# EvolvingLMMs-Lab/multimodal-sae

Measured on AMD Instinct MI355X. Metric: tokens/sec through SAE encode+TopK+decode, d=4096 width=131072, higher is better.
Workload: dtype int8 MFMA candidate select + f32 exact re-score/decode (outputs f32-exact); 1 GPU; BASELINE configs[1]: d_model=4096 width=131072 k=32, T=8192 bf16 activations/step resident in HBM, random-init unit-norm f32 weights; k=32, parallelism=single GPU, distinct_batches=4

## Files before the change

### multimodal-sae_amd/csrc/encode_fused.hip

```cpp
#include <new>
#include <cstddef>
#include <cstdlib>
#include <type_traits>

#include "common.h"
#include "gemm_mfma.h"
#include "gemm_skinny.h"
#include "encode_defs.h"
#include "encode_prep.h"
#include "encode_rescore.h"
#include "encode_small.h"
#include "encode_cert.h"

int msae_pre_acts_launch(const void *x, int x_dtype, const float *W_enc, const float *b_enc,
                         const float *b_dec, const int *rows, const int *n_rows, int T, int d, int N,
                         int relu, float *out, int ld_out, hipStream_t s);
int msae_topk_launch(const float *latents, int T, int N, int k, int ld, const int *n_rows,
                     float *vals, int32_t *idx, hipStream_t s, const TopkExtra &ex = TopkExtra());
bool msae_kth_value_launch(const float *rows, int T, int S, int ld, int r, float *out, int out_ld,
                           int out_col, hipStream_t s, const KthPush &push = KthPush());

namespace {

using GemmBf16 = GemmCfg<256, 256, 2, 2, 4, false>;
constexpr int kGemmI8Shape = MSAE_GEMM_MF == 16 ? 128 : 0;
using GemmI8 = GemmCfg<256, 256, 2, 2, 4, true, kGemmI8Shape>;
using GemmI8Cert = GemmCfg<256, 256, 2, 2, 4, true, 32 | kGemmI8Shape>;
using GemmF8 = GemmCfg<256, 256, 2, 2, 4, false, 64>;
constexpr int G_BM = GemmBf16::BM;

__global__ void zero3_i32_kernel(int *p0, size_t n0, int *p1, size_t n1, int *p2, size_t n2) {
  for (size_t i = (size_t)blockIdx.x * 256 + threadIdx.x; i < n0; i += (size_t)gridDim.x * 256) p0[i] = 0;
  for (size_t i = (size_t)blockIdx.x * 256 + threadIdx.x; i < n1; i += (size_t)gridDim.x * 256) p1[i] = 0;
  for (size_t i = (size_t)blockIdx.x * 256 + threadIdx.x; i < n2; i += (size_t)gridDim.x * 256) p2[i] = 0;
}

__global__ void zero_i32_kernel(int *p, size_t n) {
  for (size_t i = (size_t)blockIdx.x * 256 + threadIdx.x; i < n; i += (size_t)gridDim.x * 256) p[i] = 0;
}

__global__ void edit_dense_kernel(float *dense, int ld, int rows, const int *n_rows, int set_feature,
                                  float set_value, int zero_feature) {
  const int r = blockIdx.x * 256 + threadIdx.x;
  const int R = n_rows ? min(rows, *n_rows) : rows;
  if (r >= R) return;
  if (set_feature >= 0) dense[(size_t)r * ld + set_feature] = set_value;
  if (zero_feature >= 0) dense[(size_t)r * ld + zero_feature] = 0.f;
}

__global__ void iota_list_kernel(int *list, int T, int n_total) {
  const int i = blockIdx.x * 256 + threadIdx.x;
  if (i < n_total) list[i] = i < T ? i : (i == T ? T : 0);
}

__global__ void fallback_counts_kernel(const int *n_flagged, int fb_cap, int chunks, int *counts) {
  const int nf = *n_flagged;
  for (int c = threadIdx.x; c < chunks; c += blockDim.x) {
    const int left = nf - c * fb_cap;
    counts[c] = left < 0 ? 0 : (left > fb_cap ? fb_cap : left);
  }
}

struct ShardOut { unsigned char *recs; int C; int row_offset; };

constexpr int PROF_MARKS = 7;
struct ProfState {
  unsigned magic = 0x50524F46u;
  int max_steps = 0, step = 0;
  hipEvent_t *ev = nullptr;
};

inline void prof_mark(ProfState *pf, int i, hipStream_t s) {
  if (pf && pf->step < pf->max_steps) (void)hipEventRecord(pf->ev[pf->step * PROF_MARKS + i], s);
}
inline void prof_step(ProfState *pf) {
  if (pf && pf->step < pf->max_steps) ++pf->step;
}

struct FusedPlan {
  bool fast, i8, small, fm, f8;
  size_t off_fmcount, off_fmtarget, off_fmkeys, off_fmpairs, off_fmpre, off_fmdefer;
  size_t off_xhi, off_xlo, off_skeys, off_sviol, off_surv, off_sbound, off_scand, off_stau;
  int Tp, S, r, cap, r_max, fb_cap, fb_chunks;
  size_t off_rowe, off_cds, off_cds_s, off_cds_p;
  size_t off_xq, off_xqo, off_rowc, off_refs, off_colc, off_colc_s, off_colc_p, off_colmax, off_odims, off_isout, off_wqo, off_wqos;
  size_t off_xb, off_a32, off_sample, off_tauv, off_taui, off_cnt, off_cand, off_segcnt, off_segcand, off_flag, off_fbdense, off_dense, bytes;
  int segs;
};

inline FusedPlan make_plan(int T, int d, int N, int k, int mode, int shard_C = 0, bool cert = false) {
  FusedPlan p{};
  p.fast = fast_shape_ok(N, d) && T > EXACT_T_MAX && k <= 256 && k >= 1;
  if (cert && !cert_shape_ok(N, d)) p.fast = false;
  if (cert) mode = 1;
  size_t o = 0;
  auto take = [&](size_t b) { size_t at = o; o += msae_align_up(b, 256); return at; };
  if (p.fast) {
    p.Tp = (T + G_BM - 1) / G_BM * G_BM;
    p.S = N / SAMPLE_STRIDE;
    p.r = k / 8 > 16 ? k / 8 : 16;
    if (k < 32) p.r = k / 2 > 8 ? k / 2 : 8;
    if (shard_C > 0) { const int rs = shard_C / 8 > 8 ? shard_C / 8 : 8; if (rs < p.r) p.r = rs; }
    p.cap = next_pow2(128 * p.r);
    p.i8 = mode == 1 && i8_shape_ok(N, d);
    p.f8 = mode == 2 && i8_shape_ok(N, d);
    p.small = !cert && p.i8 && small_shape_ok(T, d, N, k) && getenv("MSAE_NO_SMALL_PATH") == nullptr;
    p.r_max = k <= 64 ? 8 * k : 3 * k;
    if (p.r_max < k + 4) p.r_max = k + 4;
    if (p.r_max > p.cap) p.r_max = p.cap;
    if (p.i8 || p.f8) {
      p.off_colc = take((size_t)N * 16);
      p.off_colc_s = take((size_t)p.S * 16);
      p.off_colc_p = take(p.i8 ? (size_t)N * 16 : 0);
      p.off_colmax = take((size_t)d * 4 * COLMAX_PARTS);
      p.off_odims = take((size_t)(MAX_OUT + 1) * 4);
      p.off_isout = take((size_t)d);
    }
    if (p.i8) {
      p.off_xq = take((size_t)p.Tp * d * (cert ? 2 : 1));
      p.off_xqo = take((size_t)p.Tp * MAX_OUT);
      p.off_wqo = take((size_t)N * MAX_OUT);
      p.off_wqos = take((size_t)p.S * MAX_OUT);
    }
    p.off_rowc = take((size_t)p.Tp * 16);
    p.off_rowe = take(p.i8 ? (size_t)p.Tp * 8 : 0);
    p.off_cds = take(p.i8 ? (size_t)N * 4 : 0);
    p.off_cds_s = take(p.i8 ? (size_t)p.S * 4 : 0);
    p.off_cds_p = take(p.i8 ? (size_t)N * 4 : 0);
    p.off_refs = take(256);
    if (p.small) {
      p.off_xhi = take((size_t)T * d);
      p.off_xlo = take((size_t)T * d);
      p.off_skeys = take((size_t)T * 128 * 8);
      p.off_surv = take((size_t)T * SMALL_SURV * 8);
      p.off_sbound = take((size_t)T * SMALL_GRID * 4);
      p.off_scand = take((size_t)T * 128 * 8);
      p.off_stau = take((size_t)T * 4);
      p.off_sviol = take((size_t)T * 2 * 4);
    }
    p.off_xb = take(p.i8 ? 256 : (size_t)p.Tp * d * (p.f8 ? 1 : 2));
    p.off_a32 = take((size_t)T * d * 4);
    p.off_sample = take((size_t)T * p.S * 4);
    const size_t tau_n = (size_t)T * p.r;
    p.off_tauv = take(tau_n * 4);
    p.off_taui = take(tau_n * 4);
    p.off_cnt = take((size_t)T * 4);
    p.segs = (T <= 256 && p.cap >= 1024) ? 8 : 1;
    p.off_segcnt = take(p.segs > 1 ? (size_t)T * p.segs * 4 : 0);
    p.off_cand = take((size_t)T * p.cap * 8);
    p.off_segcand = take(p.segs > 1 ? (size_t)T * p.cap * 8 : 0);
    p.fb_cap = fallback_capacity(T, N);
    p.fb_chunks = (T + p.fb_cap - 1) / p.fb_cap;
    p.off_flag = take(((size_t)T + 64 + p.fb_chunks) * 4);
    p.off_fbdense = take((size_t)p.fb_cap * N * 4);
    p.fm = shard_C == 0 && fm_shape_ok(T, k, N, d, p.r_max);
    if (p.fm) {
      p.off_fmcount = take(((size_t)N + 64 + (N + FM_SCAN_BLOCK - 1) / FM_SCAN_BLOCK) * 4);
      p.off_fmtarget = take((size_t)T * 4);
      p.off_fmkeys = take((size_t)T * p.r_max * 8);
      p.off_fmpairs = take(((size_t)T * p.r_max + (size_t)N * 16) * 8);
      p.off_fmpre = take((size_t)T * p.r_max * 4);
      p.off_fmdefer = take((size_t)T * 2 * 4);
    }
  } else {
    p.off_dense = take((size_t)T * N * 4);
  }
  p.bytes = o;
  return p;
}


template <int DT>
int run_exact_rows(const void *x, const float *W_enc, const float *b_enc, const float *b_dec, const int *list,
                   const int *n_list, int *pass_counts, float *dense, int fb_cap, int fb_chunks, int d, int N, int k,
                   int set_feature, float set_value, int zero_feature, float *vals, IdxOut idx, int32_t *status,
                   int detail, hipStream_t s) {
  if (fb_chunks > 1)
    hipLaunchKernelGGL(fallback_counts_kernel, dim3(1), dim3(64), 0, s, n_list, fb_cap, fb_chunks, pass_counts);
  for (int c = 0; c < fb_chunks; ++c) {
    const int *rows = list + (size_t)c * fb_cap, *n_rows = fb_chunks > 1 ? pass_counts + c : n_list;
    int rc = msae_pre_acts_launch(x, DT, W_enc, b_enc, b_dec, rows, n_rows, fb_cap, d, N, 1, dense, N, s);
    if (rc) return rc;
    if (set_feature >= 0 || zero_feature >= 0)
      hipLaunchKernelGGL(edit_dense_kernel, dim3((fb_cap + 255) / 256), dim3(256), 0, s, dense, N, fb_cap, n_rows,
                         set_feature, set_value, zero_feature);
    TopkExtra ex;
    ex.idx64 = idx.i64; ex.row_map = rows; ex.status = status; ex.detail = detail;
    rc = msae_topk_launch(dense, fb_cap, N, k, N, n_rows, vals, idx.i32, s, ex);
    if (rc) return rc;
  }
  return 0;
}

template <int DT>
int run_exact_fallback(const void *x, const float *W_enc, const float *b_enc, const float *b_dec, int T, int d, int N,
// ... 215 lines not shown
    hipLaunchKernelGGL(gather_wo_kernel, dim3(N / 32), dim3(256), 0, s, wq, N, d, odims,
                       reinterpret_cast<const f32x4 *>(prepared + pp.off_wstat), wqo, wqos, cc_main, cc_samp, cc_perm,
                       skip_sample ? 1 : 0, sd ? reinterpret_cast<const float *>(prepared + pp.off_ds) : (const float *)nullptr,
                       reinterpret_cast<float *>(ws + pl.off_cds), reinterpret_cast<float *>(ws + pl.off_cds_s),
                       reinterpret_cast<float *>(ws + pl.off_cds_p));
    colc = cc_main; colc_s = cc_samp;
    op_main.A = reinterpret_cast<const unsigned char *>(xq); op_main.ldA = d;
    op_main.B = skinny ? prepared + pp.off_wqf : tile_major ? prepared + pp.off_wqp : reinterpret_cast<const unsigned char *>(wq);
    op_main.ldB = d;
    op_main.nk = tile_major == 2 ? d / 64 : d / 128;
    op_main.packed = skinny ? 3 : tile_major;
    op_main.Ao = reinterpret_cast<const unsigned char *>(xqo);
    op_main.Bo = reinterpret_cast<const unsigned char *>(wqo);
    op_main.n_out = odims + MAX_OUT;
    op_samp = op_main;
    op_samp.B = skinny ? prepared + pp.off_wqsf : tile_major ? prepared + pp.off_wqsp : reinterpret_cast<const unsigned char *>(wqs);
    op_samp.Bo = reinterpret_cast<const unsigned char *>(wqos);
    if constexpr (msae_tuning::ABL_NOLEAD) { op_main.Ao = nullptr; op_main.Bo = nullptr; }
  } else if (pl.f8) {
    signed char *x8 = reinterpret_cast<signed char *>(xb);
    unsigned *colmax = reinterpret_cast<unsigned *>(ws + pl.off_colmax);
    int *odims = reinterpret_cast<int *>(ws + pl.off_odims);
    unsigned char *is_out = ws + pl.off_isout;
    f32x4 *cc_main = reinterpret_cast<f32x4 *>(ws + pl.off_colc), *cc_samp = reinterpret_cast<f32x4 *>(ws + pl.off_colc_s);
    const int ychunks = T >= 32 ? (T / 16 < 512 ? T / 16 : 512) : 1;
    hipLaunchKernelGGL((prep_colmax_kernel<DT, true>), dim3((d / 4 + 255) / 256, ychunks), dim3(256), 0, s, x, b_dec, T, d, a32,
                       colmax);
    hipLaunchKernelGGL(pick_outliers_kernel, dim3(1), dim3(1024), 0, s, colmax, d, odims, is_out);
    hipLaunchKernelGGL(quant_x_fp8_kernel, dim3(pl.Tp), dim3(256), 0, s, (const float *)a32, T, d, (const unsigned char *)is_out, x8,
                       rowc, z * z, valid);
    hipLaunchKernelGGL(gather_wo_fp8_kernel, dim3(N / 32), dim3(256), 0, s, W_enc, N, d, (const int *)odims,
                       reinterpret_cast<const f32x4 *>(prepared + pp.off_colbf), cc_main, cc_samp);
    colc = cc_main; colc_s = cc_samp;
    op_main.A = reinterpret_cast<const unsigned char *>(x8); op_main.ldA = d;
    op_main.B = prepared + pp.off_wq; op_main.ldB = d;
    op_main.nk = d / 128;
    op_main.packed = 1;
    op_samp = op_main;
    op_samp.B = prepared + pp.off_wqsp;
  } else {
    hipLaunchKernelGGL(row_p4_kernel, dim3(T), dim3(256), 0, s, a32, T, d, rowc, z * z, valid);
    colc = reinterpret_cast<const f32x4 *>(prepared + pp.off_colbf);
    colc_s = reinterpret_cast<const f32x4 *>(prepared + pp.off_colbf_s);
    op_main.A = reinterpret_cast<const unsigned char *>(xb); op_main.ldA = (size_t)d * 2;
    op_main.B = reinterpret_cast<const unsigned char *>(wb); op_main.ldB = (size_t)d * 2;
    op_main.nk = d / 64;
    op_samp = op_main;
    op_samp.B = reinterpret_cast<const unsigned char *>(wsamp);
  }

  float *refs = reinterpret_cast<float *>(ws + pl.off_refs);
  hipLaunchKernelGGL(band_refs_kernel, dim3(1), dim3(1024), 0, s, colc_s, pl.S, refs);
  prof_mark(co.prof, 1, s);
  {
    GemmEpilogue ep{};
    ep.bias = b_enc; ep.bias_stride = SAMPLE_STRIDE; ep.bias_off = SAMPLE_OFF;
    ep.dense = sample; ep.ld_dense = pl.S;
    ep.rowc = rowc; ep.colc = colc_s; ep.refs = refs; ep.zz12 = zzx;
    if (sd) { ep.row_e = reinterpret_cast<const int2 *>(ws + pl.off_rowe); ep.col_ds = reinterpret_cast<const float *>(ws + pl.off_cds_s); }
    const int grc = skinny == 64    ? gemm_skinny_launch<64, true>(op_samp, T, d, pl.S, ep, s)
                    : skinny == 128 ? gemm_skinny_launch<128, true>(op_samp, T, d, pl.S, ep, s)
                    : skinny == 256 ? gemm_skinny_launch<256, true>(op_samp, T, d, pl.S, ep, s)
                    : pl.i8         ? gemm_launch<GemmI8, true>(op_samp, T, pl.Tp, pl.S, ep, s)
                    : pl.f8         ? gemm_launch<GemmF8, true>(op_samp, T, pl.Tp, pl.S, ep, s)
                                    : gemm_launch<GemmBf16, true>(op_samp, T, pl.Tp, pl.S, ep, s);
    if (grc) return grc;
  }
  prof_mark(co.prof, 2, s);
  int rc = 0;
  const int skip_a = set_feature >= 0 ? set_feature : -1, skip_b = zero_feature >= 0 ? zero_feature : -1;
  KthPush push{};
  bool pushed = false;
  if (skip_sample && skip_a < 0 && skip_b < 0) {
    push.cnt = pcnt; push.cand = pcand; push.cap = seg_cap; push.stride = SAMPLE_STRIDE; push.off = SAMPLE_OFF;
    push.cnt_stride = pl.segs; push.row_stride = pl.cap;
    pushed = true;
  }
  if (!msae_kth_value_launch(sample, T, pl.S, pl.S, pl.r, tauv, pl.r, pl.r - 1, s, push)) {
    rc = msae_topk_launch(sample, T, pl.S, pl.r, pl.S, nullptr, tauv, taui, s);
    if (rc) return rc;
    pushed = false;
  }
  if (skip_sample && !pushed)
    hipLaunchKernelGGL(sample_push_kernel, dim3(T), dim3(256), 0, s, sample, pl.S, tauv, pl.r, pl.r - 1, skip_a, skip_b, pcnt,
                       pcand, seg_cap, pl.segs, pl.cap);
  prof_mark(co.prof, 3, s);
  const int N_main = skip_sample ? N - pl.S : N;
  {
    GemmEpilogue ep{};
    ep.bias = b_enc; ep.bias_stride = 1; ep.bias_off = 0;
    if (skip_sample) { ep.skip_stride = SAMPLE_STRIDE; ep.skip_off = SAMPLE_OFF; }
    ep.tau_vals = tauv; ep.tau_ld = pl.r; ep.tau_col = pl.r - 1;
    ep.cnt = pcnt; ep.cand = pcand; ep.cap = pl.cap; ep.segs = pl.segs;
    ep.skip_a = set_feature >= 0 ? set_feature : -1;
    ep.skip_b = zero_feature >= 0 ? zero_feature : -1;
    ep.rowc = rowc; ep.colc = skip_sample ? cc_perm : colc; ep.refs = refs; ep.zz12 = zzx;
    if (sd) {
      ep.row_e = reinterpret_cast<const int2 *>(ws + pl.off_rowe);
      ep.col_ds = reinterpret_cast<const float *>(ws + (skip_sample ? pl.off_cds_p : pl.off_cds));
    }
    if constexpr (msae_tuning::GEMM_TIMELINE != 0) {
      if (!g_timeline) (void)hipMalloc(&g_timeline, 64 * 8 * 8);
      (void)hipMemsetAsync(g_timeline, 0, 64 * 8 * 8, s);
      ep.timeline = g_timeline;
    }
    const int grc = skinny == 64    ? gemm_skinny_launch<64, false>(op_main, T, d, N_main, ep, s)
                    : skinny == 128 ? gemm_skinny_launch<128, false>(op_main, T, d, N_main, ep, s)
                    : skinny == 256 ? gemm_skinny_launch<256, false>(op_main, T, d, N_main, ep, s)
                    : pl.i8         ? gemm_launch<GemmI8, false>(op_main, T, pl.Tp, N_main, ep, s)
                    : pl.f8         ? gemm_launch<GemmF8, false>(op_main, T, pl.Tp, N, ep, s)
                                    : gemm_launch<GemmBf16, false>(op_main, T, pl.Tp, N, ep, s);
    if (grc) return grc;
  }
  if (pl.segs > 1)
    hipLaunchKernelGGL(compact_candidates_kernel, dim3(T), dim3(64), 0, s, pcnt, pcand, pl.segs, pl.cap, cnt, cand);
  prof_mark(co.prof, 4, s);
  if (shard) {
    PackArgs pa{};
    pa.cnt = cnt; pa.cand = cand; pa.cap = pl.cap;
    pa.tau_vals = tauv; pa.tau_ld = pl.r; pa.tau_col = pl.r - 1;
    pa.rowc = rowc; pa.colc = colc; pa.zz12 = zzx; pa.i8 = (pl.i8 || pl.f8) ? 1 : 0;
    pa.C = shard->C; pa.row_offset = shard->row_offset; pa.stride = shard_record_bytes(shard->C);
    pa.recs = shard->recs;
    if (pl.cap <= 64 * 32) hipLaunchKernelGGL(pack_candidates_kernel<32>, dim3(T), dim3(64), 0, s, pa);
    else if (pl.cap <= 64 * 64) hipLaunchKernelGGL(pack_candidates_kernel<64>, dim3(T), dim3(64), 0, s, pa);
    else return MSAE_ENOTIMPL;
    prof_mark(co.prof, 5, s);
    prof_mark(co.prof, 6, s);
    prof_step(co.prof);
    return msae_launch_status();
  }
// ... 561 lines not shown
```

### multimodal-sae_amd/csrc/gemm_mfma.h

```cpp
#pragma once
#include <cstdlib>

#include "common.h"
#include "tuning.h"


struct GemmEpilogue {
  const float *bias;
  int bias_stride, bias_off;
  int skip_stride, skip_off;
  float *dense; int ld_dense;
  const float *tau_vals; int tau_ld, tau_col;
  int *cnt; unsigned long long *cand; int cap;
  int segs;
  int skip_a, skip_b;
  const f32x4 *rowc, *colc;
  const float *refs;
  float zz12;
  const int2 *row_e;
  const float *col_ds;
  unsigned long long *timeline;
};

struct GemmOperands {
  const unsigned char *A, *B;
  size_t ldA, ldB;
  int nk;
  const unsigned char *Ao, *Bo;
  const int *n_out;
  int packed;
  int cert;
};

constexpr int gemm_side_bytes(int nt) { return 7 * nt * 4; }

template <bool I8_, bool F8_, bool CERT_, bool MF16_>
struct GemmEpiCfg {
  static constexpr bool I8 = I8_, F8 = F8_, CERT = CERT_, MF16 = MF16_;
  static_assert(!(I8 && F8), "fp8 accumulates in f32");
  static_assert(!MF16 || I8, "16x16x64 is an int8 shape");
  static constexpr bool SCALED = I8 || F8;
  static constexpr int BR = MF16 ? 64 : 32, BC = MF16 ? 16 : 32;
  static __device__ __forceinline__ int acc_row(int i, int e, int lane) {
    return i * BR + (MF16 ? 16 * (e >> 2) + 4 * (lane >> 4) + (e & 3) : (e & 3) + 8 * (e >> 2) + 4 * (lane >> 5));
  }
  static __device__ __forceinline__ int acc_col(int j, int lane) { return j * BC + (lane & (BC - 1)); }
};

template <int BM_, int BN_, int STAGES_, int WM_, int WN_, bool I8_ = false, int FLAGS_ = 0>
struct GemmCfg : GemmEpiCfg<I8_, (FLAGS_ & 64) != 0, (FLAGS_ & 32) != 0, (FLAGS_ & 128) != 0> {
  using GemmCfg::GemmEpiCfg::MF16;
  using GemmCfg::GemmEpiCfg::BR;
  using GemmCfg::GemmEpiCfg::BC;
  static constexpr int BM = BM_, BN = BN_, STAGES = STAGES_, WM = WM_, WN = WN_;
  static constexpr bool ABL_NOSTAGE = FLAGS_ & 4, ABL_NOREAD = FLAGS_ & 8, ABL_NOMFMA = FLAGS_ & 16;
  static constexpr int NWAVES = WM * WN, NT = NWAVES * 64;
  static constexpr int TM = BM / WM, TN = BN / WN, MI = TM / BR, NI = TN / BC;
  static constexpr int FA = MF16 ? TM / 16 : MI, FB = MF16 ? TN / 16 : NI;
  static constexpr int ROWB = 128;
  static constexpr int KS = MF16 ? 2 : 4;
  static constexpr int A_BYTES = BM * ROWB, B_BYTES = BN * ROWB, STAGE_BYTES = A_BYTES + B_BYTES;
  static constexpr int LDS_RING_BYTES = STAGES * STAGE_BYTES;
  static constexpr int SIDE_BYTES = gemm_side_bytes(NT);
  static constexpr int QCAP = 2296;
  static constexpr int LDS_BYTES = LDS_RING_BYTES + SIDE_BYTES + 16 + QCAP * 8;
  static_assert(STAGES == 2, "the flat cross-tile k-sequence below is written for a 2-slot ring");
  static_assert(BM + BN <= NT, "one thread per tile row and column fetches the epilogue constants");
  static constexpr int PIECES = STAGE_BYTES / 1024, PPW = PIECES / NWAVES;
  static constexpr int A_PIECES = A_BYTES / 1024;
  static_assert(PIECES % NWAVES == 0, "stage must split evenly over the waves");
  static_assert(TM % BR == 0 && TN % BC == 0 && TM % 32 == 0 && TN % 16 == 0, "tile shape");
  static_assert(LDS_BYTES <= 160 * 1024, "LDS budget");
};

// ... 449 lines not shown
    if constexpr (!DENSE) {
      float c5 = 0.f;
      if (tid < C::BM) {
        float b2 = r.c3 * r.ref0;
        if constexpr (C::SCALED) {
          const float rz = r.c1 * r.c1 * zz12;
          b2 = __builtin_fmaf(rz * r.c4 * r.c4, r.ref2, __builtin_fmaf(rz, r.ref1, b2));
        }
        c5 = __builtin_sqrtf(b2) * 1.00001f;
      } else if (tid < C::BM + C::BN) {
        const float q = __int_as_float(r.c2);
        float h2 = q / r.ref0;
        if constexpr (C::SCALED) {
          h2 = fmaxf(h2, r.c3 / r.ref1);
          if (r.c4 > 0.f) h2 = fmaxf(h2, r.c4 / r.ref2);
        }
        c5 = (q > 0.f || r.c3 > 0.f || r.c4 > 0.f) ? __builtin_sqrtf(h2) * 1.00001f : 0.f;
      }
      s[5 * C::NT + tid] = c5;
    }
  }
};

template <class C>
__device__ __forceinline__ float gemm_band_sq(const GemmSideView<C> &side, int row, int col, float zz12) {
  const float pz = side.P(row);
  if constexpr (!C::SCALED) return pz * side.Q(col);
  const float rs = side.sx(row), mf = side.m(row);
  const float rz = rs * rs * zz12;
  return __builtin_fmaf(pz, side.Q(col), __builtin_fmaf(rz * mf * mf, side.So(col), rz * side.Si(col)));
}

typedef float f32x2 __attribute__((ext_vector_type(2)));
template <class V>
__device__ __forceinline__ V gemm_splat(float x) {
  if constexpr (sizeof(V) == sizeof(float)) return x;
  else return V{x, x};
}
template <class C, class V>
__device__ __forceinline__ V gemm_value(const f32x16 &blk, int e, V sx, float sw, float nds, float bias) {
  V a;
  if constexpr (sizeof(V) == sizeof(float)) {
    if constexpr (C::I8) a = (float)__builtin_bit_cast(i32x16, blk)[e]; else a = blk[e];
  } else {
    if constexpr (C::I8) a = V{(float)__builtin_bit_cast(i32x16, blk)[e], (float)__builtin_bit_cast(i32x16, blk)[e + 1]};
    else a = V{blk[e], blk[e + 1]};
  }
  if constexpr (C::I8 && !C::CERT)
    return __builtin_elementwise_fma(__builtin_elementwise_fma(a, gemm_splat<V>(sw), gemm_splat<V>(nds)), sx, gemm_splat<V>(bias));
  else if constexpr (C::SCALED) return a * (sx * sw) + bias;
  else return a + bias;
}

template <class C, bool DENSE>
__device__ __forceinline__ void gemm_epilogue(f32x16 (&acc)[C::MI][C::NI], const GemmEpilogue &ep, int T,
                                              int m0, int n0, int wr, int wc, int lane,
                                              unsigned char *smem, const GemmSideView<C> side, int tl_tile = 0) {
  constexpr int QCAP = C::QCAP;
  unsigned *q_count = reinterpret_cast<unsigned *>(smem + C::LDS_RING_BYTES + C::SIDE_BYTES);
  unsigned long long *queue = reinterpret_cast<unsigned long long *>(smem + C::LDS_RING_BYTES + C::SIDE_BYTES + 16);
  asm volatile("s_waitcnt lgkmcnt(0)" ::: "memory");
  __builtin_amdgcn_s_barrier();
  if constexpr (!DENSE) {
    if (threadIdx.x == 0) *q_count = 0u;
    __syncthreads();
  }
  MSAE_TL(7);
  float c_bias[C::NI], c_sw[C::NI], c_h[C::NI];
  float c_ds[C::NI];
  bool c_live[C::NI];
#pragma unroll
  for (int j = 0; j < C::NI; ++j) {
    const int col = wc * C::TN + C::acc_col(j, lane);
    c_bias[j] = side.bias(col);
    c_sw[j] = side.sw(col);
    c_ds[j] = (C::I8 && !C::CERT) ? -side.Ds(col) : 0.f;
    c_h[j] = side.h(col);
    const int feat = gemm_feature(ep, n0 + col);
    c_live[j] = (feat != ep.skip_a) && (feat != ep.skip_b);
  }
  if (msae_tuning::ABL_NOEPI && !DENSE && ep.cap != -12345) { asm volatile("" ::"v"(acc[0][0][0])); } else
  if constexpr (!DENSE) {
    unsigned hits[C::MI][C::NI];
    constexpr int RG = C::MF16 ? 4 : 16;
#pragma unroll
    for (int i = 0; i < C::MI; ++i) {
      unsigned mj[C::NI];
#pragma unroll
      for (int j = 0; j < C::NI; ++j) mj[j] = 0u;
#pragma unroll
      for (int g = 0; g < 16 / RG; ++g) {
        if constexpr (RG < 16) __builtin_amdgcn_sched_barrier(0);
        float tau[RG], rs[RG], bt[RG];
#pragma unroll
        for (int r = 0; r < RG; ++r) {
          const int row = wr * C::TM + C::acc_row(i, RG * g + r, lane);
          tau[r] = side.tau(row);
          rs[r] = C::SCALED ? side.sx(row) : 0.f;
          bt[r] = side.B(row);
        }
#pragma unroll
        for (int j = 0; j < C::NI; ++j) {
          unsigned m = mj[j];
#pragma unroll
          for (int r = 0; r < RG; r += 2) {
            const int e = RG * g + r;
// ... 9 lines not shown
          mj[j] = m;
          if (g == 16 / RG - 1) hits[i][j] = c_live[j] ? (~m & 0xFFFFu) : 0u;
        }
      }
      if constexpr (RG < 16) __builtin_amdgcn_sched_barrier(0);
    }
    unsigned total = 0;
#pragma unroll
    for (int i = 0; i < C::MI; ++i)
#pragma unroll
      for (int j = 0; j < C::NI; ++j) total += (unsigned)__builtin_popcount(hits[i][j]);
    if (total) {
      unsigned slot;
      {
        const unsigned qa = (unsigned)(size_t)(__attribute__((address_space(3))) unsigned *)q_count;
        asm volatile("ds_add_rtn_u32 %0, %1, %2\n\ts_waitcnt lgkmcnt(0)" : "=v"(slot) : "v"(qa), "v"(total) : "memory");
      }
#pragma unroll
      for (int i = 0; i < C::MI; ++i) {
#pragma unroll
        for (int j = 0; j < C::NI; ++j) {
          unsigned h = hits[i][j];
          const int col = wc * C::TN + C::acc_col(j, lane);
          while (h) {
            const int p = 31 - __builtin_clz(h);
            h &= ~(1u << p);
            const int e = 15 - p;
            const unsigned b0 = 0u - (e & 1), b1 = 0u - ((e >> 1) & 1), b2 = 0u - ((e >> 2) & 1), b3 = 0u - ((e >> 3) & 1);
            auto sel = [](unsigned mk, unsigned hi, unsigned lo) { return (hi & mk) | (lo & ~mk); };
            unsigned s8[8], s4[4], s2[2];
#pragma unroll
            for (int q = 0; q < 8; ++q) s8[q] = sel(b0, __float_as_uint(acc[i][j][2 * q + 1]), __float_as_uint(acc[i][j][2 * q]));
#pragma unroll
            for (int q = 0; q < 4; ++q) s4[q] = sel(b1, s8[2 * q + 1], s8[2 * q]);
#pragma unroll
            for (int q = 0; q < 2; ++q) s2[q] = sel(b2, s4[2 * q + 1], s4[2 * q]);
            const float v = __uint_as_float(sel(b3, s2[1], s2[0]));
            const int row = wr * C::TM + C::acc_row(i, e, lane);
            if (slot < QCAP) {
              queue[slot] = ((unsigned long long)__float_as_uint(v) << 32) | (unsigned)(row << 16 | col);
            } else {
              const float u = v + __builtin_sqrtf(gemm_band_sq<C>(side, row, col, ep.zz12));
              if (u > side.tau(row)) {
                const int t = m0 + row;
                const int feat = gemm_feature(ep, n0 + col);
                gemm_push_candidate(ep, t, ((unsigned long long)f32_order_key(u) << 32) | (unsigned)(0x7FFFFFFF - feat));
              }
            }
            ++slot;
          }
        }
      }
    }
  } else {
#pragma unroll
    for (int i = 0; i < C::MI; ++i) {
#pragma unroll
      for (int j = 0; j < C::NI; ++j) {
        const int col = wc * C::TN + C::acc_col(j, lane);
#pragma unroll
        for (int e = 0; e < 16; ++e) {
          const int row = wr * C::TM + C::acc_row(i, e, lane), t = m0 + row;
          const float v = gemm_value<C, float>(acc[i][j], e, C::SCALED ? side.sx(row) : 0.f, c_sw[j], c_ds[j], c_bias[j]);
          if (t < T) ep.dense[(size_t)t * ep.ld_dense + n0 + col] = v + __builtin_sqrtf(gemm_band_sq<C>(side, row, col, ep.zz12));
        }
      }
    }
  }
  MSAE_TL(4);
  if constexpr (!DENSE) {
    __syncthreads();
    const unsigned nq = msae_tuning::ABL_NOFLUSH ? 0u : (*q_count < QCAP ? *q_count : QCAP);
    for (unsigned q = threadIdx.x; q < nq; q += C::NT) {
      const unsigned long long e = queue[q];
      const int row = (int)((e >> 16) & 0xFFFFu), col = (int)(e & 0xFFFFu);
      const float v = __uint_as_float((unsigned)(e >> 32));
      const float u = v + __builtin_sqrtf(gemm_band_sq<C>(side, row, col, ep.zz12));
      if (!(u > side.tau(row))) continue;
      const int t = m0 + row;
      const int feat = gemm_feature(ep, n0 + col);
      gemm_push_candidate(ep, t, ((unsigned long long)f32_order_key(u) << 32) | (unsigned)(0x7FFFFFFF - feat));
    }
  }
  MSAE_TL(5);
}

template <class C, bool DENSE>
__global__ __launch_bounds__(C::NT) void gemm_kernel(GemmOperands op, int T, int Tp, int N, int nM, int nN,
                                                     GemmEpilogue ep) {
  extern __shared__ __attribute__((aligned(1024))) unsigned char smem[];
  int seq = 0;
  [[maybe_unused]] int tl_tile = -1;
  for (int tile_id = blockIdx.x; tile_id < nM * nN; tile_id += gridDim.x) {
  ++tl_tile;
  MSAE_TL(0);
  int tid_ = threadIdx.x;
  asm volatile("" : "+v"(tid_));
  const int lane = tid_ & 63;
  const int wave = __builtin_amdgcn_readfirstlane(tid_ >> 6);
  const int wr = wave / C::WN, wc = wave % C::WN;
  int tm, tn;
  gemm_map_tile(tile_id, nM, nN, tm, tn);
  const int m0 = tm * C::BM, n0 = tn * C::BN;
  const bool has_next = tile_id + (int)gridDim.x < nM * nN;
  int m0n = 0, n0n = 0;
  if (has_next) {
// ... 171 lines not shown
```

### multimodal-sae_amd/csrc/topk.hip

```cpp
#include "common.h"

namespace {

constexpr int TK_THREADS = 1024;
constexpr int TK_WAVES = TK_THREADS / 64;
constexpr int TK_BINS = 4096;

struct TkShared {
  unsigned hist[TK_BINS];
  unsigned wave_tot[TK_WAVES];
  unsigned bin;
  unsigned remaining;
  unsigned base_gt;
  unsigned base_eq;
};

__device__ __forceinline__ unsigned wave_incl_scan(unsigned v, int lane) {
#pragma unroll
  for (int off = 1; off < 64; off <<= 1) {
    unsigned n = __shfl_up(v, off, 64);
    if (lane >= off) v += n;
  }
  return v;
}
// ... 192 lines not shown
  {
    unsigned mx = 0u;
#pragma unroll
    for (int i = 0; i < VPL; ++i) mx = key[i] > mx ? key[i] : mx;
#pragma unroll
    for (int off = 32; off > 0; off >>= 1) { const unsigned o = __shfl_xor(mx, off, 64); mx = o > mx ? o : mx; }
    const unsigned pre = mx & 0xFF000000u;
    int c = 0;
#pragma unroll
    for (int i = 0; i < VPL; ++i) c += (key[i] >= pre) ? 1 : 0;
#pragma unroll
    for (int off = 32; off > 0; off >>= 1) c += __shfl_xor(c, off, 64);
    if (c >= r) { lo = pre; first_bit = 23; }
  }
#pragma unroll 1
  for (int bit = first_bit; bit >= KTH_LOW_BIT; --bit) {
    const unsigned mid = lo | (1u << bit);
    int c = 0;
#pragma unroll
    for (int i = 0; i < VPL; ++i) c += (key[i] >= mid) ? 1 : 0;
#pragma unroll
    for (int off = 32; off > 0; off >>= 1) c += __shfl_xor(c, off, 64);
    if (c >= r) lo = mid;
  }
  if (lane == 0) out[(size_t)t * out_ld + out_col] = f32_from_order_key(lo);
  if (push.cnt && f32_from_order_key(lo) > 0.f) {
    int total = 0;
#pragma unroll
    for (int i = 0; i < VPL; ++i) {
      total += __builtin_popcountll(__builtin_amdgcn_ballot_w64(key[i] > lo));
      if ((i & 7) == 7) asm volatile("" : "+s"(total));
    }
    if (total == 0) return;
    int base = 0;
    if (lane == 0) base = atomicAdd(push.cnt + (size_t)t * push.cnt_stride, total);
    base = __builtin_amdgcn_readfirstlane(base);
    unsigned long long *list = push.cand + (size_t)t * (push.row_stride ? push.row_stride : push.cap);
    unsigned lo2 = lo;
    asm volatile("" : "+v"(lo2));
#pragma unroll
    for (int i = 0; i < VPL; ++i) {
      const bool hit = key[i] > lo2;
      const unsigned long long m = __builtin_amdgcn_ballot_w64(hit);
      if (m == 0ull) continue;
      if (hit) {
        const int slot = base + (int)__builtin_amdgcn_mbcnt_hi((unsigned)(m >> 32), __builtin_amdgcn_mbcnt_lo((unsigned)m, 0u));
        const int j = ((i >> 2) * 64 + lane) * 4 + (i & 3);
        unsigned kk;
        asm volatile("v_mov_b32 %0, %1" : "=v"(kk) : "v"(key[i]));
        if (slot < push.cap) list[slot] = ((unsigned long long)kk << 32) | (unsigned)(0x7FFFFFFF - (j * push.stride + push.off));
      }
      base += __builtin_popcountll(m);
      if ((i & 7) == 7) asm volatile("" : "+s"(base));
    }
  }
}

__global__ __launch_bounds__(64) void merge_topk_kernel(const int32_t *__restrict__ gathered, int T,
                                                        int G, int kl, int k,
                                                        float *__restrict__ vals,
                                                        int32_t *__restrict__ idx,
                                                        int32_t *__restrict__ flagged) {
  extern __shared__ __attribute__((aligned(16))) unsigned long long mkeys[];
  const int lane = threadIdx.x, t = blockIdx.x;
  const int M = G * kl, np = next_pow2(M);
  unsigned long long worst_last = 0ull;
  for (int i = lane; i < np; i += 64) {
    unsigned long long key = 0ull;
    if (i < M) {
      const int g = i / kl, j = i % kl;
      const float v = __int_as_float(gathered[(((size_t)g * 2 + 0) * T + t) * kl + j]);
      const int f = gathered[(((size_t)g * 2 + 1) * T + t) * kl + j];
      key = rank_key(v, f);
      if (j == kl - 1) worst_last = key > worst_last ? key : worst_last;
    }
    mkeys[i] = key;
  }
#pragma unroll
  for (int off = 32; off > 0; off >>= 1) {
    const unsigned long long o = __shfl_xor(worst_last, off, 64);
    worst_last = o > worst_last ? o : worst_last;
  }
  for (int size = 2; size <= np; size <<= 1)
    for (int stride = size >> 1; stride > 0; stride >>= 1) {
      __syncthreads();
      for (int i = lane; i < (np >> 1); i += 64) {
        const int lo = (i / stride) * (stride << 1) + (i % stride), hi = lo + stride;
        const bool desc = ((lo & size) == 0);
        const unsigned long long x = mkeys[lo], y = mkeys[hi];
        if ((x < y) == desc) { mkeys[lo] = y; mkeys[hi] = x; }
      }
    }
  __syncthreads();
  for (int j = lane; j < k; j += 64) {
    const unsigned long long key = mkeys[j];
    idx[(size_t)t * k + j] = rank_key_index(key);
    vals[(size_t)t * k + j] = f32_from_order_key((unsigned)(key >> 32));
  }
  if (lane == 0 && flagged) flagged[t] = (kl < k && worst_last >= mkeys[k - 1]) ? 1 : 0;
}

__global__ __launch_bounds__(1024) void compact_flags_kernel(const int32_t *__restrict__ flags, int T,
                                                             int32_t *__restrict__ rows, int32_t *__restrict__ n_rows) {
  __shared__ int wsum[16];
  __shared__ int s_base;
  const int tid = threadIdx.x, lane = tid & 63, wv = tid >> 6;
// ... 44 lines not shown
        const bool desc = ((lo & size) == 0);
        const unsigned long long x = mkeys[lo], y = mkeys[hi];
        if ((x < y) == desc) { mkeys[lo] = y; mkeys[hi] = x; }
      }
    }
  __syncthreads();
  for (int j = lane; j < k; j += 64) {
    const unsigned long long key = mkeys[j];
    if (idx) idx[(size_t)t * k + j] = rank_key_index(key);
    if (idx64) idx64[(size_t)t * k + j] = rank_key_index(key);
    vals[(size_t)t * k + j] = f32_from_order_key((unsigned)(key >> 32));
  }
}

}

extern "C" size_t msae_topk_ws_bytes(int T, int N, int k) {
  (void)T; (void)N; (void)k;
  return 0;
}

int msae_topk_launch(const float *latents, int T, int N, int k, int ld, const int *n_rows,
                     float *vals, int32_t *idx, hipStream_t s, const TopkExtra &ex) {
  if (T < 0 || N <= 0 || k <= 0 || k > N || k > 16384 || ld < N) return MSAE_EINVAL;
  if (T == 0) return 0;
  const size_t smem = sizeof(TkShared) + (size_t)next_pow2(k) * sizeof(unsigned long long);
  const bool vec = (N % 4 == 0) && (ld % 4 == 0) && msae_aligned(latents, 16);
  if (smem > 48 * 1024) {
    if (vec) MSAE_HIP_TRY(hipFuncSetAttribute((const void *)topk_rows_kernel<true>, hipFuncAttributeMaxDynamicSharedMemorySize, (int)smem));
    else MSAE_HIP_TRY(hipFuncSetAttribute((const void *)topk_rows_kernel<false>, hipFuncAttributeMaxDynamicSharedMemorySize, (int)smem));
  }
  const int grid = (n_rows && T > 128) ? 128 : T;
  if (vec)
    hipLaunchKernelGGL(topk_rows_kernel<true>, dim3(grid), dim3(TK_THREADS), smem, s, latents, T, N, k, ld,
                       n_rows, vals, idx, ex);
  else
    hipLaunchKernelGGL(topk_rows_kernel<false>, dim3(grid), dim3(TK_THREADS), smem, s, latents, T, N, k,
                       ld, n_rows, vals, idx, ex);
  return msae_launch_status();
}

bool msae_kth_value_launch(const float *rows, int T, int S, int ld, int r, float *out, int out_ld,
                           int out_col, hipStream_t s, const KthPush &push) {
  if (S % 256 || ld % 4 || !msae_aligned(rows, 16) || r < 1 || r > S) return false;
  const dim3 grid((T + 3) / 4), block(256);
  switch (S / 64) {
#define KTH_CASE(V) case V: hipLaunchKernelGGL(kth_value_kernel<V>, grid, block, 0, s, rows, T, S, ld, r, out, out_ld, out_col, push); return true;
    KTH_CASE(4) KTH_CASE(8) KTH_CASE(16) KTH_CASE(32) KTH_CASE(64) KTH_CASE(128)
#undef KTH_CASE
    default: return false;
  }
}

extern "C" int msae_topk_f32(const float *latents, int T, int N, int k, float *vals, int32_t *idx,
                             void *ws, size_t ws_bytes, void *stream) {
  (void)ws; (void)ws_bytes;
  return msae_topk_launch(latents, T, N, k, N, nullptr, vals, idx, (hipStream_t)stream, TopkExtra());
}

extern "C" int msae_merge_topk(const int32_t *gathered, int T, int G, int kl, int k, float *vals,
                               int32_t *idx, int32_t *flagged, void *stream) {
  if (T < 0 || G <= 0 || kl <= 0 || k <= 0 || (long)G * kl < k || (long)G * kl > 8192) return MSAE_EINVAL;
  if (T == 0) return 0;
  const size_t smem = (size_t)next_pow2(G * kl) * sizeof(unsigned long long);
  MSAE_HIP_TRY(hipFuncSetAttribute((const void *)merge_topk_kernel,
                                   hipFuncAttributeMaxDynamicSharedMemorySize, (int)smem));
  hipLaunchKernelGGL(merge_topk_kernel, dim3(T), dim3(64), smem, (hipStream_t)stream, gathered, T, G,
                     kl, k, vals, idx, flagged);
  return msae_launch_status();
}

extern "C" int msae_compact_flags(const int32_t *flags, int T, int32_t *rows, int32_t *n_rows, void *stream) {
  if (T < 0 || !rows || !n_rows || (T > 0 && !flags)) return MSAE_EINVAL;
  hipLaunchKernelGGL(compact_flags_kernel, dim3(1), dim3(1024), 0, (hipStream_t)stream, flags, T, rows, n_rows);
  return msae_launch_status();
}

extern "C" int msae_merge_topk_masked(const int32_t *gathered, int T, int G, int kl, int k, const int32_t *mask,
                                      float *vals, int32_t *idx, int64_t *idx64, void *stream) {
  if (T < 0 || G <= 0 || kl <= 0 || k <= 0 || (long)G * kl < k || (long)G * kl > 8192 || !mask || !vals || (!idx && !idx64))
    return MSAE_EINVAL;
  if (T == 0) return 0;
  const size_t smem = (size_t)next_pow2(G * kl) * sizeof(unsigned long long);
  MSAE_HIP_TRY(hipFuncSetAttribute((const void *)merge_topk_masked_kernel,
                                   hipFuncAttributeMaxDynamicSharedMemorySize, (int)smem));
  hipLaunchKernelGGL(merge_topk_masked_kernel, dim3(T), dim3(64), smem, (hipStream_t)stream, gathered, T, G, kl, k, mask,
                     vals, idx, idx64);
  return msae_launch_status();
}
```

Before: 1.578 million tokens/s.

## Compact per-tile top-R keys in sample GEMM epilogue instead of dense sample matrix

In the int8 sample GEMM epilogue, each 256-column tile now does a radix select per row. It writes only the top-R keys plus a bound on the discarded keys, instead of storing the full dense sample row. A new kth_compact kernel then selects the r-th threshold from the compacted keys, clamps it by the max discarded bound, and pushes candidates. This cuts the dense sample write and the later full read and select. The cost is extra LDS staging and syncthreads inside the GEMM epilogue, and a threshold that may be looser than before.

```diff
diff --git a/multimodal-sae_amd/csrc/encode_fused.hip b/multimodal-sae_amd/csrc/encode_fused.hip
--- a/multimodal-sae_amd/csrc/encode_fused.hip
+++ b/multimodal-sae_amd/csrc/encode_fused.hip
@@ -19,6 +19,8 @@
                      float *vals, int32_t *idx, hipStream_t s, const TopkExtra &ex = TopkExtra());
 bool msae_kth_value_launch(const float *rows, int T, int S, int ld, int r, float *out, int out_ld,
                            int out_col, hipStream_t s, const KthPush &push = KthPush());
+bool msae_kth_compact_launch(const unsigned long long *ktop, const unsigned *kbound, int T, int n_tiles, int R, int r, float *out,
+                             int out_ld, int out_col, hipStream_t s, const KthPush &push);
 
 namespace {
 
@@ -86,6 +88,8 @@
   size_t off_xq, off_xqo, off_rowc, off_refs, off_colc, off_colc_s, off_colc_p, off_colmax, off_odims, off_isout, off_wqo, off_wqos;
   size_t off_xb, off_a32, off_sample, off_tauv, off_taui, off_cnt, off_cand, off_segcnt, off_segcand, off_flag, off_fbdense, off_dense, bytes;
   int segs;
+  size_t off_ktop, off_kbound;
+  int kR;
 };
 
 inline FusedPlan make_plan(int T, int d, int N, int k, int mode, int shard_C = 0, bool cert = false) {
@@ -141,6 +145,10 @@
     p.off_xb = take(p.i8 ? 256 : (size_t)p.Tp * d * (p.f8 ? 1 : 2));
     p.off_a32 = take((size_t)T * d * 4);
     p.off_sample = take((size_t)T * p.S * 4);
+    p.kR = p.r <= 16 ? 16 : (p.r <= 32 ? 32 : 0);
+    if (!p.i8 || cert || p.S % 256 || p.S / 256 * p.kR > 1024) p.kR = 0;
+    p.off_ktop = take(p.kR ? (size_t)T * (p.S / 256) * p.kR * 8 : 0);
+    p.off_kbound = take(p.kR ? (size_t)T * (p.S / 256) * 4 : 0);
     const size_t tau_n = (size_t)T * p.r;
     p.off_tauv = take(tau_n * 4);
     p.off_taui = take(tau_n * 4);
@@ -462,10 +470,16 @@
   float *refs = reinterpret_cast<float *>(ws + pl.off_refs);
   hipLaunchKernelGGL(band_refs_kernel, dim3(1), dim3(1024), 0, s, colc_s, pl.S, refs);
   prof_mark(co.prof, 1, s);
+  const int skip_a = set_feature >= 0 ? set_feature : -1, skip_b = zero_feature >= 0 ? zero_feature : -1;
+  const bool compact = GemmI8::MF16 && pl.i8 && pl.kR > 0 && skinny == 0 && skip_sample && skip_a < 0 && skip_b < 0 &&
+                       getenv("MSAE_DENSE_SAMPLE") == nullptr;
+  unsigned long long *ktop = reinterpret_cast<unsigned long long *>(ws + pl.off_ktop);
+  unsigned *kbound = reinterpret_cast<unsigned *>(ws + pl.off_kbound);
   {
     GemmEpilogue ep{};
     ep.bias = b_enc; ep.bias_stride = SAMPLE_STRIDE; ep.bias_off = SAMPLE_OFF;
     ep.dense = sample; ep.ld_dense = pl.S;
+    if (compact) { ep.ktop = ktop; ep.kbound = kbound; ep.ktop_r = pl.kR; }
     ep.rowc = rowc; ep.colc = colc_s; ep.refs = refs; ep.zz12 = zzx;
     if (sd) { ep.row_e = reinterpret_cast<const int2 *>(ws + pl.off_rowe); ep.col_ds = reinterpret_cast<const float *>(ws + pl.off_cds_s); }
     const int grc = skinny == 64    ? gemm_skinny_launch<64, true>(op_samp, T, d, pl.S, ep, s)
@@ -478,7 +492,6 @@
   }
   prof_mark(co.prof, 2, s);
   int rc = 0;
-  const int skip_a = set_feature >= 0 ? set_feature : -1, skip_b = zero_feature >= 0 ? zero_feature : -1;
   KthPush push{};
   bool pushed = false;
   if (skip_sample && skip_a < 0 && skip_b < 0) {
@@ -486,7 +499,9 @@
     push.cnt_stride = pl.segs; push.row_stride = pl.cap;
     pushed = true;
   }
-  if (!msae_kth_value_launch(sample, T, pl.S, pl.S, pl.r, tauv, pl.r, pl.r - 1, s, push)) {
+  if (compact) {
+    if (!msae_kth_compact_launch(ktop, kbound, T, pl.S / 256, pl.kR, pl.r, tauv, pl.r, pl.r - 1, s, push)) return MSAE_EINVAL;
+  } else if (!msae_kth_value_launch(sample, T, pl.S, pl.S, pl.r, tauv, pl.r, pl.r - 1, s, push)) {
     rc = msae_topk_launch(sample, T, pl.S, pl.r, pl.S, nullptr, tauv, taui, s);
     if (rc) return rc;
     pushed = false;
diff --git a/multimodal-sae_amd/csrc/gemm_mfma.h b/multimodal-sae_amd/csrc/gemm_mfma.h
--- a/multimodal-sae_amd/csrc/gemm_mfma.h
+++ b/multimodal-sae_amd/csrc/gemm_mfma.h
@@ -20,6 +20,9 @@
   const int2 *row_e;
   const float *col_ds;
   unsigned long long *timeline;
+  unsigned long long *ktop;
+  unsigned *kbound;
+  int ktop_r;
 };
 
 struct GemmOperands {
@@ -575,6 +578,84 @@
   else return a + bias;
 }
 
+template <class C>
+__device__ __forceinline__ void gemm_compact_rows(f32x16 (&acc)[C::MI][C::NI], const GemmEpilogue &ep, int T, int m0, int n0,
+                                                  int wr, int wc, int lane, unsigned char *smem, const GemmSideView<C> side) {
+  constexpr int CH = 16, STR = C::BN + 4;
+  static_assert(C::MF16 && C::BN == 256 && C::NWAVES * 2 == CH && CH * STR * 4 <= C::QCAP * 8,
+                "16x16x64 blocks, 4 keys per lane and row, two rows per wave, the chunk inside the queue region");
+  unsigned *kb = reinterpret_cast<unsigned *>(smem + C::LDS_RING_BYTES + C::SIDE_BYTES + 16);
+  const int R = ep.ktop_r, n_tiles = ep.ld_dense / C::BN, b = n0 / C::BN;
+  const int wave = wr * C::WN + wc;
+#pragma unroll
+  for (int i = 0; i < C::MI; ++i) {
+#pragma unroll
+    for (int g = 0; g < 4; ++g) {
+#pragma unroll 1
+      for (int h = 0; h < C::WM; ++h) {
+        __syncthreads();
+        if (wr == h) {
+#pragma unroll
+          for (int j = 0; j < C::NI; ++j) {
+            const int col = wc * C::TN + C::acc_col(j, lane);
+            const float sw = side.sw(col), nds = -side.Ds(col), bias = side.bias(col);
+#pragma unroll
+            for (int q = 0; q < 4; ++q) {
+              const int e = 4 * g + q, row = wr * C::TM + C::acc_row(i, e, lane);
+              const float v = gemm_value<C, float>(acc[i][j], e, side.sx(row), sw, nds, bias);
+              kb[(row & (CH - 1)) * STR + col] = f32_order_key(v + __builtin_sqrtf(gemm_band_sq<C>(side, row, col, ep.zz12)));
+            }
+          }
+        }
+        __syncthreads();
+#pragma unroll 1
+        for (int rr = 0; rr < 2; ++rr) {
+          unsigned key[4], lo = 0u;
+          {
+            const u32x4 k4 = *reinterpret_cast<const u32x4 *>(kb + (2 * wave + rr) * STR + lane * 4);
+#pragma unroll
+            for (int q = 0; q < 4; ++q) key[q] = k4[q];
+          }
+#pragma unroll 1
+          for (int bit = 31; bit >= 14; --bit) {
+            const unsigned mid = lo | (1u << bit);
+            int c = 0;
+#pragma unroll
+            for (int q = 0; q < 4; ++q) c += __builtin_popcountll(__builtin_amdgcn_ballot_w64(key[q] >= mid));
+            if (c >= R) lo = mid;
+          }
+          const int row = h * C::TM + 64 * i + 16 * g + 2 * wave + rr, t = m0 + row;
+          const unsigned gp = lo >> 14;
+          int n_above = 0;
+#pragma unroll
+          for (int q = 0; q < 4; ++q) n_above += __builtin_popcountll(__builtin_amdgcn_ballot_w64((key[q] >> 14) > gp));
+          const int need = R - n_above;
+          unsigned long long *dst = ep.ktop + ((size_t)t * n_tiles + b) * R;
+          int n_grp = 0, n_kept = 0;
+          unsigned dmax = 0u;
+#pragma unroll
+          for (int q = 0; q < 4; ++q) {
+            const unsigned p = key[q] >> 14;
+            const unsigned long long mg = __builtin_amdgcn_ballot_w64(p == gp);
+            const int grank = n_grp + (int)__builtin_amdgcn_mbcnt_hi((unsigned)(mg >> 32), __builtin_amdgcn_mbcnt_lo((unsigned)mg, 0u));
+            n_grp += __builtin_popcountll(mg);
+            const bool keep = p > gp || (p == gp && grank < need);
+            const unsigned long long mk = __builtin_amdgcn_ballot_w64(keep);
+            const int slot = n_kept + (int)__builtin_amdgcn_mbcnt_hi((unsigned)(mk >> 32), __builtin_amdgcn_mbcnt_lo((unsigned)mk, 0u));
+            n_kept += __builtin_popcountll(mk);
+            if (keep && t < T)
+              dst[slot] = ((unsigned long long)key[q] << 32) | (unsigned)(0x7FFFFFFF - gemm_feature(ep, n0 + lane * 4 + q));
+            if (!keep) dmax = key[q] > dmax ? key[q] : dmax;
+          }
+#pragma unroll
+          for (int off = 32; off > 0; off >>= 1) { const unsigned o = __shfl_xor(dmax, off, 64); dmax = o > dmax ? o : dmax; }
+          if (lane == 0 && t < T) ep.kbound[(size_t)t * n_tiles + b] = dmax | 0x3FFFu;
+        }
+      }
+    }
+  }
+}
+
 template <class C, bool DENSE>
 __device__ __forceinline__ void gemm_epilogue(f32x16 (&acc)[C::MI][C::NI], const GemmEpilogue &ep, int T,
                                               int m0, int n0, int wr, int wc, int lane,
@@ -690,6 +771,8 @@
         }
       }
     }
+  } else if (C::MF16 && !C::CERT && ep.ktop != nullptr) {
+    if constexpr (C::MF16 && !C::CERT) gemm_compact_rows<C>(acc, ep, T, m0, n0, wr, wc, lane, smem, side);
   } else {
 #pragma unroll
     for (int i = 0; i < C::MI; ++i) {
diff --git a/multimodal-sae_amd/csrc/topk.hip b/multimodal-sae_amd/csrc/topk.hip
--- a/multimodal-sae_amd/csrc/topk.hip
+++ b/multimodal-sae_amd/csrc/topk.hip
@@ -268,6 +268,74 @@
       }
       base += __builtin_popcountll(m);
       if ((i & 7) == 7) asm volatile("" : "+s"(base));
+    }
+  }
+}
+
+template <int VPL>
+__global__ __launch_bounds__(256) void kth_compact_kernel(const unsigned long long *__restrict__ ktop,
+                                                          const unsigned *__restrict__ kbound, int T, int n_tiles, int R,
+                                                          int r, float *__restrict__ out, int out_ld, int out_col, KthPush push) {
+  const int lane = threadIdx.x & 63;
+  const int t = blockIdx.x * 4 + (threadIdx.x >> 6);
+  if (t >= T) return;
+  const int M = n_tiles * R;
+  const unsigned long long *row = ktop + (size_t)t * M;
+  unsigned long long kk[VPL];
+  unsigned key[VPL];
+#pragma unroll
+  for (int i = 0; i < VPL; ++i) {
+    const int j = i * 64 + lane;
+    kk[i] = j < M ? row[j] : 0ull;
+    key[i] = (unsigned)(kk[i] >> 32);
+  }
+  unsigned B = 0u;
+  for (int j = lane; j < n_tiles; j += 64) { const unsigned v = kbound[(size_t)t * n_tiles + j]; B = v > B ? v : B; }
+#pragma unroll
+  for (int off = 32; off > 0; off >>= 1) { const unsigned o = __shfl_xor(B, off, 64); B = o > B ? o : B; }
+  unsigned lo = 0u;
+  int first_bit = 31;
+  {
+    unsigned mx = 0u;
+#pragma unroll
+    for (int i = 0; i < VPL; ++i) mx = key[i] > mx ? key[i] : mx;
+#pragma unroll
+    for (int off = 32; off > 0; off >>= 1) { const unsigned o = __shfl_xor(mx, off, 64); mx = o > mx ? o : mx; }
+    const unsigned pre = mx & 0xFF000000u;
+    int c = 0;
+#pragma unroll
+    for (int i = 0; i < VPL; ++i) c += __builtin_popcountll(__builtin_amdgcn_ballot_w64(key[i] >= pre));
+    if (c >= r) { lo = pre; first_bit = 23; }
+  }
+#pragma unroll 1
+  for (int bit = first_bit; bit >= KTH_LOW_BIT; --bit) {
+    const unsigned mid = lo | (1u << bit);
+    int c = 0;
+#pragma unroll
+    for (int i = 0; i < VPL; ++i) c += __builtin_popcountll(__builtin_amdgcn_ballot_w64(key[i] >= mid));
+    if (c >= r) lo = mid;
+  }
+  const unsigned thr = lo >= B ? lo : B;
+  const float tau = f32_from_order_key(thr);
+  if (lane == 0) out[(size_t)t * out_ld + out_col] = tau;
+  if (push.cnt && tau > 0.f) {
+    int total = 0;
+#pragma unroll
+    for (int i = 0; i < VPL; ++i) total += __builtin_popcountll(__builtin_amdgcn_ballot_w64(key[i] > thr));
+    if (total == 0) return;
+    int base = 0;
+    if (lane == 0) base = atomicAdd(push.cnt + (size_t)t * push.cnt_stride, total);
+    base = __builtin_amdgcn_readfirstlane(base);
+    unsigned long long *list = push.cand + (size_t)t * (push.row_stride ? push.row_stride : push.cap);
+#pragma unroll
+    for (int i = 0; i < VPL; ++i) {
+      const bool hit = key[i] > thr;
+      const unsigned long long m = __builtin_amdgcn_ballot_w64(hit);
+      if (hit) {
+        const int slot = base + (int)__builtin_amdgcn_mbcnt_hi((unsigned)(m >> 32), __builtin_amdgcn_mbcnt_lo((unsigned)m, 0u));
+        if (slot < push.cap) list[slot] = kk[i];
+      }
+      base += __builtin_popcountll(m);
     }
   }
 }
@@ -418,6 +486,20 @@
   }
 }
 
+bool msae_kth_compact_launch(const unsigned long long *ktop, const unsigned *kbound, int T, int n_tiles, int R, int r, float *out,
+                             int out_ld, int out_col, hipStream_t s, const KthPush &push) {
+  const int M = n_tiles * R;
+  if (r < 1 || R < r || n_tiles < 1 || M > 1024) return false;
+  const dim3 grid((T + 3) / 4), block(256);
+  const int vpl = M <= 64 ? 1 : M <= 128 ? 2 : M <= 256 ? 4 : M <= 512 ? 8 : 16;
+  switch (vpl) {
+#define KTHC_CASE(V) case V: hipLaunchKernelGGL(kth_compact_kernel<V>, grid, block, 0, s, ktop, kbound, T, n_tiles, R, r, out, out_ld, out_col, push); return true;
+    KTHC_CASE(1) KTHC_CASE(2) KTHC_CASE(4) KTHC_CASE(8) KTHC_CASE(16)
+#undef KTHC_CASE
+    default: return false;
+  }
+}
+
 extern "C" int msae_topk_f32(const float *latents, int T, int N, int k, float *vals, int32_t *idx,
                              void *ws, size_t ws_bytes, void *stream) {
   (void)ws; (void)ws_bytes;
```

New measurement: 1.524 million tokens/s. 3.4% lower.
